# comfy-creator/Comfy-Gen-Server

Measured on AMD Instinct MI355X. Metric: images/sec (whole node) + sec/image, SDXL 1024 20-step Euler-a at 1/2/4/8 MI355X, higher is better.
Workload: dtype bf16; 1 GPU; model=sdxl-base, global_batch=8, seq_len=16384, resolution=1024, sampler_steps=20, sampler=euler_ancestral, unet_batch_per_gpu=16, parallelism=dp1, pipelined=True

## Files before the change

comfy_gen_server_amd/_native.py:

```python
from __future__ import annotations

import ctypes
import glob
import os
import threading

_HERE = os.path.dirname(os.path.abspath(__file__))
LIB_DIR = os.path.join(_HERE, "lib")
_lock = threading.Lock()
_kernels = None
_kernels_err = None


def kernel_lib_path() -> str:
    return os.environ.get("CGS_KERNELS_SO") or os.path.join(LIB_DIR, "libcgs_kernels.so")


def load_kernels():
    global _kernels, _kernels_err
    if _kernels is not None or _kernels_err is not None:
        return _kernels
    with _lock:
        if _kernels is not None or _kernels_err is not None:
            return _kernels
# ... 100 lines not shown
    "cgs_step_param": [_P, _I, _P, _I, _I, _P, _P],
    "cgs_step_advance": [_P, _P],
    "cgs_vae_out_u8": [_P, _P, _L, _P],
    "cgs_conv2d_nhwc_ex": [_P, _P, _I, _P, _P, _P, _P, _I, _I, _I, _I, _I, _I, _I, _I, _I, _I, _I, _I, _P],
    "cgs_region_accumulate": [_P, _P, _P, _I, _P, _I, _I, _I, _I, _I, _I, _I, _I, _I, _L, _L, _L, _L, _I, _L, _L,
                              _L, _L, _I, _F, _P],
    "cgs_region_normalize": [_P, _P, _P, _L, _I, _P],
    "cgs_clip_embed": [_P, _P, _P, _P, _I, _I, _I, _I, _I, _P],
    "cgs_pooled_gather": [_P, _P, _P, _I, _I, _I, _I, _P],
    "cgs_layernorm_stats": [_P, _P, _I, _I, _F, _I, _P],
    "cgs_gemm_bf16_lnfold": [_P, _P, _P, _P, _P, _P, _I, _I, _I, _L, _L, _L, _I, _P, _L, _P],
    "cgs_gemm_bf16_lnfold_v": [_P, _P, _P, _P, _P, _P, _I, _I, _I, _L, _L, _L, _I, _P, _L, _I, _P],
    "cgs_v7_ws_bytes": [_I, _I, _I],
    "cgs_v7_set_dbg": [_I],
    "cgs_v6_set_mode": [_I],
    "cgs_attn_set_prio": [_I],
    "cgs_gn_set_blocks": [_I],
    "cgs_conv_smalln_set_lds": [_I],
    "cgs_attn_set_kv2_rows": [_I],
    "cgs_grn_set_rows": [_I],
    "cgs_flash_attn_fwd_ks": [_P, _P, _P, _P, _I, _I, _I, _I, _L, _L, _L, _L, _L, _L, _L, _L, _F, _I, _P, _P, _P],
    "cgs_flash_attn_fwd_kv2": [_P, _P, _P, _P, _P, _P, _I, _I, _I, _I, _I, _L, _L, _L, _L, _L, _L, _L, _L, _L, _L, _L, _L, _F, _P],
    "cgs_conv2d_nhwc_gns": [_P, _P, _I, _P, _P, _P, _P, _I, _I, _I, _I, _I, _I, _I, _I, _I, _I, _I, _I, _P, _P],
    "cgs_groupnorm_band_stats": [_P, _P, _I, _P, _P, _P, _I, _I, _I, _I, _I, _P],
    "cgs_groupnorm_apply_stats": [_P, _P, _I, _P, _P, _P, _P, _P, _P, _I, _I, _I, _I, _I, _I, _P],
    "cgs_groupnorm_nhwc_part": [_P, _P, _P, _P, _P, _P, _P, _I, _I, _I, _I, _I, _F, _I, _I, _P],
    "cgs_groupnorm_nhwc_part_pld": [_P, _P, _P, _P, _P, _I, _P, _P, _I, _I, _I, _I, _I, _F, _I, _I, _P],
    "cgs_groupnorm_nhwc_ws_pld": [_P, _P, _P, _P, _P, _I, _P, _I, _I, _I, _I, _F, _I, _I, _P],
    "cgs_groupnorm_nhwc_dual_pld": [_P, _P, _I, _P, _P, _P, _P, _I, _P, _I, _I, _I, _I, _F, _I, _I, _P],
    "cgs_gemm_bf16_v7ws": [_P, _P, _P, _P, _P, _I, _I, _I, _L, _L, _L, _L, _I, _F, _P, _L, _P],
    "cgs_conv2d_nhwc_v7ws": [_P, _P, _I, _P, _P, _P, _P, _I, _I, _I, _I, _I, _I, _I, _I, _I, _I, _I, _I, _P, _L, _P],
    "cgs_fourier_filter": [_P, _P, _P, _I, _I, _I, _I, _L, _L, _L, _L, _L, _L, _L, _L, _I, _F, _I, _P],
    "cgs_tome_match": [_P, _P, _P, _P, _P, _I, _I, _I, _I, _L, _L, _L, _L, _I, _P],
    "cgs_grn_nhwc_v2": [_P, _P, _P, _P, _P, _I, _I, _I, _I, _I, _P],
    "cgs_grn_slices": [_I, _I, _I],
    "cgs_bgemm_f32": [_P, _P, _P, _I, _I, _I, _I, _L, _L, _L, _L, _L, _L, _L, _L, _F, _I, _I, _P],
    "cgs_softmax2_f32_bf16": [_P, _P, _L, _I, _L, _L, _P],
    "cgs_transpose_bf16": [_P, _P, _I, _I, _L, _L, _P],
    "cgs_abort_stream_capture": [_P],
    "cgs_channel_affine2": [_P, _P, _P, _L, _P, _I, _I, _I, _F, _I, _P],
    "cgs_gemm_bf16_w6": [_P, _P, _P, _P, _P, _P, _P, _I, _I, _I, _L, _L, _L, _L, _I, _F, _I, _I, _I, _I, _P],
    "cgs_gemm_w6_ok": [_I, _I, _I, _L, _L, _L, _L, _I, _I],
    "cgs_gemm_skinny_ws": [_P, _P, _P, _P, _P, _I, _I, _I, _L, _L, _L, _L, _I, _F, _P, _L, _P],
    "cgs_gemm_skinny_ws_bytes": [_I, _I, _I],
    "cgs_gemm_bf16_rowstats": [_P, _P, _P, _P, _P, _I, _I, _I, _L, _L, _L, _L, _I, _F, _P, _P],
    "cgs_gemm_bf16_rowstats_v": [_P, _P, _P, _P, _P, _I, _I, _I, _L, _L, _L, _L, _I, _F, _P, _I, _P],
# ... 54 lines not shown
```

comfy_gen_server_amd/csrc/kernels/conv.hip:

```cpp
#include "common.h"
#include <stdlib.h>
#include "mfma_core.h"
#include "mfma_pp.h"
#include "mfma_pp160.h"
#include "mfma_ppk.h"

#define EPI_BIAS 1
#define EPI_RESIDUAL 2
#define CONV_UP2X 16
#ifndef CGS_CONV_PFE
#define CGS_CONV_PFE 0
#endif

typedef __attribute__((address_space(3))) void lds_void;

__device__ __attribute__((aligned(16))) unsigned char g_conv_zero_page[256];

struct ConvArgs {
  const u16* in;
  const u16* in2;
  const u16* w;
  const u16* bias;
  const u16* res;
  u16* out;
  int N, H, W, Cin, C1, Cout, kh, kw, stride, pad, Ho, Wo;
  int flags;
  int tiles_n;
// ... 417 lines not shown
        for (int kx = 0; kx < a->kw; ++kx)
          if (ry && (unsigned)(px + kx) < (unsigned)a->W) m |= 1u << (ky * a->kw + kx);
      }
    }
    vm[s] = m;
    const unsigned ch = 16u * (unsigned)pp::src_chunk8(s & 1);
    pb1[s] = pix * (2u * (unsigned)a->C1) + ch;
    pb2[s] = pix * (2u * (unsigned)(a->Cin - a->C1)) + ch;
  }
  __device__ __forceinline__ void dma(int s, int k0, unsigned char* dst) const {
    const unsigned kq = (unsigned)k0 >> 6;
    const unsigned tap = __umulhi(kq, a->cq_magic) + (a->cq_magic ? 0u : kq);
    const int ci0 = k0 - (int)tap * a->Cin;
    const int ky = (int)((tap * (unsigned)a->kw_m16) >> 16);
    const int kx = (int)tap - ky * a->kw;
    const bool second = ci0 >= a->C1;
    const unsigned cs2 = 2u * (unsigned)(second ? a->Cin - a->C1 : a->C1);
    const unsigned so = (unsigned)(ky * a->W + kx) * cs2 + 2u * (unsigned)(second ? ci0 - a->C1 : ci0);
    const unsigned off = ((second ? pb2[s] : pb1[s]) + so) | (~(vm[s] << (31u - tap)) & 0x80000000u);
    __builtin_amdgcn_raw_ptr_buffer_load_lds(second ? r2 : r1, (lds_void*)dst, 16, off, 0, 0, 0);
  }
};

struct ConvGatherKU {
  static constexpr bool kOwnDMA = true;
  const ConvArgs* a;
  uint32_t pb[4], vm[4];
  int py[4], px[4];
  __amdgpu_buffer_rsrc_t r1;
  __device__ __forceinline__ void make(long long n_img, unsigned pixels) {
    r1 = __builtin_amdgcn_make_buffer_rsrc((void*)(a->in + n_img * pixels * a->C1), 0,
                                           (int)(pixels * (unsigned)a->C1 * 2u), 0x00020000);
  }
  __device__ __forceinline__ void init() {
    if (!a->img_rsrc) make(0, (unsigned)(a->N * a->H * a->W));
  }
  __device__ __forceinline__ void tile(int m0) {
    if (a->img_rsrc) make(m0 / (a->Ho * a->Wo), (unsigned)(a->H * a->W));
  }
  __device__ __forceinline__ void setup(int s, int row) {
    const int M = a->N * a->Ho * a->Wo;
    const bool ok = row < M;
    row = ok ? row : M - 1;
    const int hw = a->Ho * a->Wo;
    const int n = row / hw;
    const int rem = row - n * hw;
// ... 139 lines not shown
  conv_magic(a);
  if (g_conv_v6_ld != 1 && kd) conv_run<conv_nhwc_v5k_kernel<true>>(a, nwg, pp::THREADS, pp::LDS, stream);
  else conv_run<conv_nhwc_v5k_kernel<false>>(a, nwg, pp::THREADS, pp::LDS, stream);
}

static int conv_pq_loader(ConvArgs& a) {
  const int kd = conv_kd(a);
  int ld = conv_fast_ok(a) ? (kd ? 2 : 1) : ((a.flags & CONV_UP2X) && kd ? 3 : 0);
  if (g_conv_v6_ld >= 0 && g_conv_v6_ld < ld) ld = ld == 3 ? 0 : g_conv_v6_ld;
  a.img_rsrc = ld >= 2 && kd == 2;
  if (ld) conv_magic(a);
  return ld;
}
template <typename F>
static void with_loader(int ld, F f) {
  if (ld == 3) f(std::integral_constant<int, 3>{});
  else if (ld == 2) f(std::integral_constant<int, 2>{});
  else if (ld == 1) f(std::integral_constant<int, 1>{});
  else f(std::integral_constant<int, 0>{});
}

template <int LD>
using ConvLoaderFor = typename std::conditional<
    LD == 3, ConvGatherKU,
    typename std::conditional<LD == 2, ConvGatherKD,
                              typename std::conditional<LD == 1, ConvGatherK<true>, ConvGatherA8>::type>::type>::type;
template <int LD, int DS = 0, bool GNS = false, int NJ = 5, int PFE = CGS_CONV_PFE>
__global__ __launch_bounds__(512) __attribute__((amdgpu_waves_per_eu(2, 2))) void conv_nhwc_v6_kernel(ConvArgs a) {
  extern __shared__ __attribute__((aligned(16))) unsigned char smem[];
  const int M = a.N * a.Ho * a.Wo;
  const int K = a.kh * a.kw * a.Cin;
  ConvLoaderFor<LD> al;
  al.a = &a;
  if constexpr (LD >= 2) al.init();
  mc::Epi e = conv_epi(a);
  e.gnp = a.gnp;
  e.hw = a.Ho * a.Wo;
  pq::run<decltype(al), false, DS, GNS, false, false, false, PFE, NJ>(al, a.w, K, M, a.Cout, K, e, smem,
                                                                              (M + pq::BM - 1) / pq::BM, a.tiles_n,
                                                                              a.group_m);
}

template <int LD>
__global__ __launch_bounds__(256) __attribute__((amdgpu_waves_per_eu(2, 2))) void conv_nhwc_v6w4_kernel(ConvArgs a) {
  extern __shared__ __attribute__((aligned(16))) unsigned char smem[];
  const int M = a.N * a.Ho * a.Wo;
  const int K = a.kh * a.kw * a.Cin;
  ConvLoaderFor<LD> al;
  al.a = &a;
// ... 25 lines not shown
  if (a.gnp) n128 = false;
  const long long T = conv_tiles(a, pq::BM, n128 ? pq::Geo<4>::BN : pq::BN);
  const int grid = (int)(T < num_cus() ? T : num_cus());
  const int ds = v6_conv_ds();
  with_loader(conv_pq_loader(a), [&](auto lc) {
    constexpr int L = decltype(lc)::value;
    if (a.gnp) {
      conv_v6_launch<L, 51, true>(a, grid, stream);
      return;
    }
    if (n128) {
      conv_v6_launch<L, 51, false, 4, 0>(a, grid, stream);
      return;
    }
    switch (ds) {
      case 0: conv_v6_launch<L, 0>(a, grid, stream); break;
      case 3: conv_v6_launch<L, 3>(a, grid, stream); break;
      case 17: conv_v6_launch<L, 17>(a, grid, stream); break;
      case 19: conv_v6_launch<L, 19>(a, grid, stream); break;
      case 1: conv_v6_launch<L, 1>(a, grid, stream); break;
      default: conv_v6_launch<L, 51>(a, grid, stream);
    }
  });
}

template <int LOADER>
__global__ __launch_bounds__(512) __attribute__((amdgpu_waves_per_eu(2, 2))) void conv_nhwc_v7_kernel(ConvArgs a) {
  extern __shared__ __attribute__((aligned(16))) unsigned char smem[];
  const int M = a.N * a.Ho * a.Wo;
  const int K = a.kh * a.kw * a.Cin;
  typename std::conditional<LOADER == 2, ConvGatherKL,
                            typename std::conditional<LOADER == 1, ConvGatherKB, ConvGatherA8>::type>::type al;
  al.a = &a;
  if constexpr (LOADER >= 1) al.init();
  mc::Epi e = conv_epi(a);
  ppk::run<false>(al, a.w, K, M, a.Cout, K, e, smem, (M + ppk::BM - 1) / ppk::BM, a.tiles_n, a.group_m, a.sp);
}

static void conv_v7_go(ConvArgs& a, hipStream_t stream, void* ws = nullptr, long long ws_bytes = 0) {
  const int K = a.kh * a.kw * a.Cin;
  const long long T = conv_tiles(a, ppk::BM, ppk::BN);
  a.sp = ppk::Split{0, 1, nullptr, nullptr, 0};
  long long U = T;
  if (ws && ws_bytes >= ppk::split_ws_bytes(T, K / ppk::BK, num_cus())) {
    a.sp.S = ppk::split_plan(T, K / ppk::BK, num_cus(), a.sp.t_full);
    if (a.sp.S > 1) {
// ... 217 lines not shown
static bool smalln_lds() {
  if (g_smalln_lds < 0) g_smalln_lds = getenv("CGS_SMALLN_LDS") ? atoi(getenv("CGS_SMALLN_LDS")) != 0 : 1;
  return g_smalln_lds != 0;
}
CGS_EXPORT void cgs_conv_smalln_set_lds(int on) { g_smalln_lds = on != 0; }

static int conv_smalln_launch(const ConvArgs& a, hipStream_t stream) {
  const long long nwg = (long long)a.N * ((a.Ho + 15) / 16) * ((a.Wo + 15) / 16);
  if (nwg > 0x7fffffffLL || nwg < 1) return (int)hipErrorInvalidValue;
  if (smalln_lds() && a.kh == 3 && a.kw == 3 && a.stride == 1 && a.pad == 1 && !(a.flags & CONV_UP2X) &&
      a.in2 == nullptr && a.Cin % 32 == 0 && a.Ho == a.H && a.Wo == a.W && a.Cout <= 16 &&
      (long long)a.H * a.W * a.Cin < (1ll << 31)) {
    conv_nhwc_smalln_lds_kernel<<<(unsigned)nwg, 256, 0, stream>>>(a);
    return (int)hipGetLastError();
  }
  if (a.kh == 3 && a.kw == 3) conv_nhwc_smalln_kernel<3><<<(unsigned)nwg, 256, 0, stream>>>(a);
  else if (a.kh == 1 && a.kw == 1) conv_nhwc_smalln_kernel<1><<<(unsigned)nwg, 256, 0, stream>>>(a);
  else conv_nhwc_smalln_kernel<0><<<(unsigned)nwg, 256, 0, stream>>>(a);
  return (int)hipGetLastError();
}

static int conv_launch(ConvArgs& a, hipStream_t stream, int variant = -2, void* ws = nullptr, long long ws_bytes = 0) {
  if (variant == -2) variant = g_conv_variant;
  if (a.Cout <= 16 && (variant != 2 || a.Cin % 64 || (a.in2 && a.C1 % 64))) return conv_smalln_launch(a, stream);
  if (variant != 2 && a.Cout % 8 == 0) return conv_v3_launch(a, variant, stream, ws, ws_bytes);
  if (a.Cout >= 1024) conv_run<conv_nhwc_v2_kernel<256>>(a, conv_tiles(a, 256, 256), 512, 4 * 64 * (256 + 256), stream);
  else conv_run<conv_nhwc_v2_kernel<128>>(a, conv_tiles(a, 256, 128), 512, 4 * 64 * (256 + 128), stream);
  return (int)hipGetLastError();
}

static ConvArgs conv_args(const void* x, const void* x2, int C1, const void* w, const void* bias, const void* res,
                          void* out, int N, int H, int W, int Cin, int Cout, int kh, int kw, int stride, int pad,
                          int Ho, int Wo, int flags) {
  return ConvArgs{(const u16*)x, (const u16*)x2, (const u16*)w, (const u16*)bias, (const u16*)res, (u16*)out, N, H, W,
                  Cin, x2 ? C1 : Cin, Cout, kh, kw, stride, pad, Ho, Wo,
                  (bias ? EPI_BIAS : 0) | (res ? EPI_RESIDUAL : 0) | (flags & CONV_UP2X), 0, g_conv_group};
}

static bool conv_shape_ok(const ConvArgs& a) {
  return !(a.Cin % 32 || (a.in2 && a.C1 % 32) || a.Cout < 1 ||
           (a.Cout % 8 && a.Cout > 16 && (a.Cin % 64 || (a.in2 && a.C1 % 64))));
}

CGS_EXPORT int cgs_conv2d_nhwc(const void* x, const void* w, const void* bias, const void* res, void* out, int N, int H,
                               int W, int Cin, int Cout, int kh, int kw, int stride, int pad, int Ho, int Wo,
                               hipStream_t stream) {
// ... 19 lines not shown
                                   const void* res, void* out, int N, int H, int W, int Cin, int Cout, int kh, int kw,
                                   int stride, int pad, int Ho, int Wo, int flags, int variant, int act,
                                   float act_param, hipStream_t stream) {
  ConvArgs a = conv_args(x, x2, C1, w, bias, res, out, N, H, W, Cin, Cout, kh, kw, stride, pad, Ho, Wo, flags);
  if (!conv_shape_ok(a) || Cout <= 16 || Cout % 8 || (variant != 3 && variant != 4 && variant != 8) ||
      act < CGS_ACT_NONE || act > CGS_ACT_LEAKY_RELU)
    return (int)hipErrorInvalidValue;
  a.act = act;
  a.act_param = act_param;
  return conv_launch(a, stream, variant);
}

CGS_EXPORT int cgs_conv2d_nhwc_gns(const void* x, const void* x2, int C1, const void* w, const void* bias,
                                   const void* res, void* out, int N, int H, int W, int Cin, int Cout, int kh, int kw,
                                   int stride, int pad, int Ho, int Wo, int flags, float* gnp, hipStream_t stream) {
  ConvArgs a = conv_args(x, x2, C1, w, bias, res, out, N, H, W, Cin, Cout, kh, kw, stride, pad, Ho, Wo, flags);
  if (!gnp || ((uintptr_t)gnp % 16) || (Ho * Wo) % 256 || Cout % 8 || !conv_variant_ok(a, 6))
    return (int)hipErrorInvalidValue;
  a.gnp = gnp;
  conv_v6_go(a, stream);
  return (int)hipGetLastError();
}

CGS_EXPORT int cgs_conv2d_nhwc_v7ws(const void* x, const void* x2, int C1, const void* w, const void* bias,
                                    const void* res, void* out, int N, int H, int W, int Cin, int Cout, int kh, int kw,
                                    int stride, int pad, int Ho, int Wo, int flags, void* ws, long long ws_bytes,
                                    hipStream_t stream) {
  ConvArgs a = conv_args(x, x2, C1, w, bias, res, out, N, H, W, Cin, Cout, kh, kw, stride, pad, Ho, Wo, flags);
  return conv_shape_ok(a) ? conv_launch(a, stream, 7, ws, ws_bytes) : (int)hipErrorInvalidValue;
}
```

comfy_gen_server_amd/csrc/kernels/mfma_pp160.h:

```cpp
#pragma once
#include "common.h"
#include "mfma_core.h"
#include "mfma_pp.h"

namespace pq {

typedef uint32_t u32x4v __attribute__((ext_vector_type(4)));
typedef uint32_t u32x2v __attribute__((ext_vector_type(2)));
__device__ __forceinline__ void untracked_load(u32x4v& d, const void* p) {
  asm volatile("global_load_dwordx4 %0, %1, off" : "=v"(d) : "v"(p));
}
__device__ __forceinline__ void untracked_load(u32x2v& d, const void* p) {
  asm volatile("global_load_dwordx2 %0, %1, off" : "=v"(d) : "v"(p));
}

constexpr int BM = 256, BN = 160, BK = 64;
constexpr int THREADS = 512;
constexpr int A_BYTES = BM * 128;
constexpr int B_BYTES = BN * 128;
constexpr int STAGE = A_BYTES + B_BYTES;
constexpr int LDS = 3 * STAGE;
template <int NJ, int NI = 4, int W = 8>
struct Geo {
  static constexpr int GW = 16 * NJ, BN = GW * (W / 4);
  static constexpr int BM = 64 * NI;
  static constexpr int PR = 8 * W;
  static constexpr int NA = BM / PR;
  static constexpr int A_BYTES = BM * 128;
  static constexpr int B_BYTES = BN * 128, STAGE = A_BYTES + B_BYTES, LDS = 3 * STAGE;
  static constexpr int NBG = (BN + PR - 1) / PR;
  static constexpr int REM = BN % PR;
  static constexpr bool B_HALF = REM != 0;
};

template <int NJ = 5>
__device__ __forceinline__ int b_col160(int r) {
  constexpr int GW = 16 * NJ;
  const int g = r >= GW, l = r - GW * g, j = l >> 4, q = l & 15;
  if (j >= 4) return GW * g + 64 + q;
  return GW * g + 32 * (j >> 1) + 8 * (q >> 2) + 4 * (j & 1) + (q & 3);
// ... 85 lines not shown
#pragma unroll
        for (int g = 0; g < 4; ++g) dma_a(g, kt, slot);
      } else {
#pragma unroll
        for (int g = 0; g < 3; ++g) dma_b(g, kt, slot);
      }
    } else {
      if (part == 0) {
        dma_a(0, kt, slot);
        dma_a(1, kt, slot);
        dma_b(0, kt, slot);
      } else {
        dma_a(2, kt, slot);
        dma_a(3, kt, slot);
        dma_b(1, kt, slot);
        dma_b(2, kt, slot);
      }
    }
  };
  auto stage = [&](int kt, int slot) {
    stage_part(0, kt, slot);
    if constexpr ((DS & 3) != 0) stage_part(1, kt, slot);
  };
  auto wait_tile = [&]() {
    if (!Gm::B_HALF || wave < Gm::REM / 8) mc::wait_vmcnt<Gm::NA + Gm::NBG>();
    else mc::wait_vmcnt<Gm::NA + Gm::NBG - 1>();
  };

  f32x4 acc[NI][NJ];
  const int fr = lane & 15, fq = lane >> 4;
  bf16x8 af[NI], bfr[NJ];
  auto read_frags = [&](const unsigned char* S, int kk) {
#pragma unroll
    for (int i = 0; i < NI; ++i) {
      const int r = wm * (16 * NI) + 16 * i + fr;
      const int c = (4 * kk + fq) ^ ((r >> 1) & 7);
      af[i] = *reinterpret_cast<const bf16x8*>(S + r * 128 + 16 * c);
    }
    const unsigned char* SB = S + A_BYTESv;
#pragma unroll
    for (int j = 0; j < NJ; ++j) {
      const int r = grp * GW + 16 * j + fr;
      const int c = (4 * kk + fq) ^ ((r >> 1) & 7);
      bfr[j] = *reinterpret_cast<const bf16x8*>(SB + r * 128 + 16 * c);
    }
  };
  auto mma = [&]() {
// ... 292 lines not shown
  using T0 = std::false_type;
  using T1 = std::true_type;
  auto epilogue = [&](int m0, int n0) {
    if constexpr (LN) {
      if (hb) epilogue_t(m0, n0, T1{}, T0{});
      else epilogue_t(m0, n0, T0{}, T0{});
      return;
    }
    if (hr) {
      if (hb) epilogue_t(m0, n0, T1{}, T1{});
      else epilogue_t(m0, n0, T0{}, T1{});
    } else {
      if (hb) epilogue_t(m0, n0, T1{}, T0{});
      else epilogue_t(m0, n0, T0{}, T0{});
    }
  };

  int l = base_l;
  int m0, n0;
  coords(l, m0, n0);
  setup(m0, n0);
  stage(0, 0);
  stage(nk > 1 ? 1 : 0, 1);
  wait_tile();
  pp::barrier();
  if (NW == 8 && grp == 1) pp::barrier();

  int slot = 0;
  while (true) {
    const int ln = l + G;
    const bool has_next = ln < T;
    int nm0 = 0, nn0 = 0;
    if (has_next) coords(ln, nm0, nn0);
#pragma unroll
    for (int i = 0; i < NI; ++i)
#pragma unroll
      for (int j = 0; j < NJ; ++j) acc[i][j] = f32x4{0.f, 0.f, 0.f, 0.f};
    auto ktile = [&](int kt, bool PF) {
      const unsigned char* S = smem + slot * STAGE;
      const int slot2 = slot >= 1 ? slot - 1 : 2;
      const int kst = kt + 2 < nk ? kt + 2 : (has_next ? kt + 2 - nk : nk - 1);
      if (kt + 2 == nk && has_next) setup(nm0, nn0);
      if constexpr ((DS & 4) != 0) stage_part(0, kst, slot2);
      read_frags(S, 0);
      if constexpr ((DS & 4) == 0) stage_part(0, kst, slot2);
      if constexpr ((DS & 16) == 0) pp::wait_lgkm0();
      pp::barrier();
      mma();
      pp::barrier();
      if constexpr ((DS & 4) != 0) stage_part(1, kst, slot2);
      read_frags(S, 1);
      if constexpr ((DS & 4) == 0) stage_part(1, kst, slot2);
      wait_tile();
      if (PFE && PF) prefetch(m0, n0, hb, PFE == 1 && hr);
      pp::wait_lgkm0();
      pp::barrier();
      mma();
      pp::barrier();
      slot = slot == 2 ? 0 : slot + 1;
    };
    if constexpr (PFE == 2) {
      for (int kt = 0; kt < nk; ++kt) ktile(kt, kt == nk - 2);
    } else if constexpr (PFE) {
      for (int kt = 0; kt < nk - 2; ++kt) ktile(kt, false);
      ktile(nk - 2, true);
      ktile(nk - 1, false);
    } else {
      for (int kt = 0; kt < nk; ++kt) ktile(kt, false);
    }
    epilogue(m0, n0);
    if (!has_next) break;
    l = ln;
    m0 = nm0;
    n0 = nn0;
  }
  if (NW == 8 && grp == 0) pp::barrier();
// ... 5 lines not shown
```

comfy_gen_server_amd/ops/core.py:

```python
from __future__ import annotations

import collections
import math
import os

import numpy as np
import torch
import torch.nn.functional as F

from .. import _native
from . import autotune
from . import f32 as _f32
from .dispatch import backend_for, count, vendor_fallback

_DT = {torch.float32: 0, torch.bfloat16: 1, torch.float16: 2}

EPI_BIAS = 1
EPI_RESIDUAL = 2
EPI_GEGLU = 4
EPI_SILU_IN = 8
EPI_LNFOLD = 8
EPI_GELU = 32
EPI_F32OUT = 16

# ... 790 lines not shown
    pd = padding[0] if isinstance(padding, (tuple, list)) else padding
    y = sc.conv2d(lambda xx, _: _conv2d(xx, weight, bias, st, pd, None, weight_nhwc, groups, upsample2x, None),
                  x, weight.shape[2], st, pd, upsample2x, x2)
    if residual is not None:
        y = y + residual
    return y.contiguous(memory_format=torch.channels_last) if y.is_cuda else y


def upconv_tap_weights(weight: torch.Tensor) -> torch.Tensor:
    Cout, Cin = weight.shape[:2]
    G = (Cout + 15) // 16
    w = weight.new_zeros((G * 16, Cin, 9))
    w[:Cout] = weight.reshape(Cout, Cin, 9)
    return w.view(G, 16, Cin, 9).permute(0, 3, 1, 2).contiguous().view(G * 144, Cin)


def _upconv_use_taps(N, H, W, Cin, Cout, cached) -> bool:
    mode = os.environ.get("CGS_UPCONV_TAPS", "")
    if mode in ("0", "1"):
        return mode == "1"
    return cached and Cin >= 256 and Cout >= 32 and N * H * W * Cin * Cout * 36 >= (1 << 27)


CONV_VARIANTS = {"v2": 2, "v3": 3, "v4": 4, "v5": 5, "v6": 6, "v7": 7, "v8": 8, "v6n128": 18, "v6w4": 21, "auto": -2}
_FUSED_ACT_CONV = ("v3", "v4", "v8")


def _conv_operands(xc, x2c, w_nhwc, bias, res, out, kh, kw, stride, pad, flags):
    N, C1, H, W = xc.shape
    _, Cout, Ho, Wo = out.shape
    return (xc.data_ptr(), _ptr(x2c), C1, w_nhwc.data_ptr(), _ptr(bias), _ptr(res), out.data_ptr(), N, H, W,
            C1 + (0 if x2c is None else x2c.shape[1]), Cout, kh, kw, stride, pad, Ho, Wo, flags)


def _conv2d_act(x, weight, bias, stride, padding, residual, weight_nhwc, groups, upsample2x, x2, act, act_param):
    if act not in ACT_CODES:
        raise ValueError(f"unknown activation {act!r} (one of {sorted(ACT_CODES)})")
    st = stride[0] if isinstance(stride, (tuple, list)) else stride
    pd = padding[0] if isinstance(padding, (tuple, list)) else padding

    def split():
        y = conv2d(x, weight, bias, st, pd, weight_nhwc=weight_nhwc, groups=groups, upsample2x=upsample2x, x2=x2)
        y = activation(y, act, act_param, inplace=True)
        return y if residual is None else y + residual.to(y.dtype)

    Cout, _, kh, kw = weight.shape
    C1 = x.shape[1]
# ... 62 lines not shown
        x2c = None if x2 is None else x2.contiguous(memory_format=torch.channels_last)
        Hl, Wl = (2 * H, 2 * W) if upsample2x else (H, W)
        Ho = (Hl + 2 * padding - kh) // stride + 1
        Wo = (Wl + 2 * padding - kw) // stride + 1
        xc = x.contiguous(memory_format=torch.channels_last)
        r = None
        if residual is not None:
            r = residual.contiguous(memory_format=torch.channels_last)
        flags = 16 if upsample2x else 0

        def run(variant):
            out = torch.empty((N, Cout, Ho, Wo), device=x.device, dtype=x.dtype,
                              memory_format=torch.channels_last)
            pre = _conv_operands(xc, x2c, weight_nhwc, bias, r, out, kh, kw, stride, padding, flags)
            ws = _v7_ws(N * Ho * Wo, Cout, kh * kw * Cin, x.device) if variant == 7 else None
            if ws is not None:
                _check(_lib().cgs_conv2d_nhwc_v7ws(*pre, ws.data_ptr(), ws.numel(), _stream()), "cgs_conv2d_nhwc_v7ws")
            else:
                _check(_lib().cgs_conv2d_nhwc_v(*pre, variant, _stream()), "cgs_conv2d_nhwc")
            return out

        variant = -2
        M = N * Ho * Wo
        if M * Cout * Cin * kh * kw >= (1 << 27) and Cout > 16:
            cands = [("v4", lambda: run(4))]
            if Cout % 8 == 0:
                cands.append(("v8", lambda: run(8)))
            if Cin % 64 == 0:
                cands += [("v7", lambda: run(7)), ("v5", lambda: run(5)), ("v6", lambda: run(6)),
                          ("v2", lambda: run(2))]
                if Cout % 128 == 0 and Cout % 160 and kh * kw * Cin >= 128:
                    cands.append(("v6n128", lambda: run(18)))
                if Cout % 80 == 0 and kh * kw * Cin >= 128 and M <= 32768:
                    cands.append(("v6w4", lambda: run(21)))
            choice = autotune.choose(("conv", N, H, W, Cin, Cout, kh, stride, padding, flags, int(r is not None))
                                     + ((("dual", C1),) if x2c is not None else ()), cands, default="auto")
            variant = CONV_VARIANTS[choice]
        if (upsample2x and single and r is None and not gn_stats and kh == 3 and kw == 3 and stride == 1
                and padding == 1 and Cout % 8 == 0 and weight.dtype == x.dtype
                and _native.has_kernel("cgs_upconv_taps_nhwc")):
            def run_taps():
                wt = weight_taps() if callable(weight_taps) else weight_taps
                if wt is None:
                    wt = upconv_tap_weights(weight)
                out = torch.empty((N, Cout, Ho, Wo), device=x.device, dtype=x.dtype,
                                  memory_format=torch.channels_last)
                _check(_lib().cgs_upconv_taps_nhwc(xc.data_ptr(), wt.data_ptr(), _ptr(bias), out.data_ptr(), N, H, W,
                                                   Cin, Cout, _stream()), "cgs_upconv_taps_nhwc")
                return out

            if _upconv_use_taps(N, H, W, Cin, Cout, weight_taps is not None):
                return run_taps()
        if (gn_stats and variant == 6 and _GNS and (Ho * Wo) % 256 == 0 and Cin % 64 == 0 and C1 % 64 == 0
                and Cout % 8 == 0 and kh * kw * Cin >= 128 and (bias is None or bias.data_ptr() % 8 == 0)
                and _native.has_kernel("cgs_conv2d_nhwc_gns")):
            out = torch.empty((N, Cout, Ho, Wo), device=x.device, dtype=x.dtype, memory_format=torch.channels_last)
            part = torch.empty(N * (Ho * Wo // 64) * Cout * 2, device=x.device, dtype=torch.float32)
            _check(_lib().cgs_conv2d_nhwc_gns(*_conv_operands(xc, x2c, weight_nhwc, bias, r, out, kh, kw, stride,
                                                              padding, flags), part.data_ptr(), _stream()),
                   "cgs_conv2d_nhwc_gns")
            out._cgs_gnpart = (part, out.data_ptr())
            return out
        return run(variant)
    if upsample2x:
        x = upsample_nearest2x(x)
    if be == "torch":
        count("conv", "torch")
        y = F.conv2d(x.float(), weight.float(), None if bias is None else bias.float(), stride, padding,
                     groups=groups)
        if residual is not None:
            y = y + residual.float()
        return y.to(x.dtype)
    vendor_fallback("conv", f"dtype {x.dtype}, groups={groups}, Cin={x.shape[1]}, Cout={Cout}")
    y = F.conv2d(x, weight, bias, stride, padding, groups=groups)
    if residual is not None:
        y = y + residual
    return y


_CT_TAPS = ((3, 1), (2, 0))


def conv_transpose_phase_weights(weight: torch.Tensor):
# ... 1308 lines not shown
```

Before: 3.465 images/s.

## Add halo-patch 3x3 conv kernel reusing LDS input tile across all nine taps

Adds a new v6p conv kernel for 3x3 stride-1 convolutions. It loads an 18x18 halo input patch per channel slab into LDS once and reuses it for all nine taps, instead of re-gathering the im2col A operand for every tap. Weight tiles for each tap are streamed through a triple-buffered slot ring, and the kernel supports the fused GroupNorm partial-stats epilogue. It is enabled by default for a fixed set of SDXL UNet shapes whenever variant 6 is chosen, and it is also added as an autotune candidate. A probe loader variant that skips A loads after the first tap is also added, but it is not on the default path.

```diff
diff --git a/comfy_gen_server_amd/_native.py b/comfy_gen_server_amd/_native.py
--- a/comfy_gen_server_amd/_native.py
+++ b/comfy_gen_server_amd/_native.py
@@ -146,6 +146,8 @@
     "cgs_flash_attn_fwd_ks": [_P, _P, _P, _P, _I, _I, _I, _I, _L, _L, _L, _L, _L, _L, _L, _L, _F, _I, _P, _P, _P],
     "cgs_flash_attn_fwd_kv2": [_P, _P, _P, _P, _P, _P, _I, _I, _I, _I, _I, _L, _L, _L, _L, _L, _L, _L, _L, _L, _L, _L, _L, _F, _P],
     "cgs_conv2d_nhwc_gns": [_P, _P, _I, _P, _P, _P, _P, _I, _I, _I, _I, _I, _I, _I, _I, _I, _I, _I, _I, _P, _P],
+    "cgs_conv2d_nhwc_gns_v": [_P, _P, _I, _P, _P, _P, _P, _I, _I, _I, _I, _I, _I, _I, _I, _I, _I, _I, _I, _P, _I, _P],
+    "cgs_conv2d_nhwc_probe": [_P, _P, _P, _P, _P, _I, _I, _I, _I, _I, _I, _I, _I, _I, _I, _I, _P],
     "cgs_groupnorm_band_stats": [_P, _P, _I, _P, _P, _P, _I, _I, _I, _I, _I, _P],
     "cgs_groupnorm_apply_stats": [_P, _P, _I, _P, _P, _P, _P, _P, _P, _I, _I, _I, _I, _I, _I, _P],
     "cgs_groupnorm_nhwc_part": [_P, _P, _P, _P, _P, _P, _P, _I, _I, _I, _I, _I, _F, _I, _I, _P],
diff --git a/comfy_gen_server_amd/csrc/kernels/conv.hip b/comfy_gen_server_amd/csrc/kernels/conv.hip
--- a/comfy_gen_server_amd/csrc/kernels/conv.hip
+++ b/comfy_gen_server_amd/csrc/kernels/conv.hip
@@ -3,6 +3,7 @@
 #include "mfma_core.h"
 #include "mfma_pp.h"
 #include "mfma_pp160.h"
+#include "mfma_pp160p.h"
 #include "mfma_ppk.h"
 
 #define EPI_BIAS 1
@@ -466,6 +467,14 @@
   }
 };
 
+struct ConvGatherKD1 : ConvGatherKD {
+  static constexpr bool kTapProbe = true;
+  __device__ __forceinline__ bool has_a(int k0) const { return k0 < a->Cin; }
+  __device__ __forceinline__ void dma(int s, int k0, unsigned char* dst) const {
+    if (has_a(k0)) ConvGatherKD::dma(s, k0, dst);
+  }
+};
+
 struct ConvGatherKU {
   static constexpr bool kOwnDMA = true;
   const ConvArgs* a;
@@ -651,9 +660,10 @@
 
 template <int LD>
 using ConvLoaderFor = typename std::conditional<
+    LD == 4, ConvGatherKD1, typename std::conditional<
     LD == 3, ConvGatherKU,
     typename std::conditional<LD == 2, ConvGatherKD,
-                              typename std::conditional<LD == 1, ConvGatherK<true>, ConvGatherA8>::type>::type>::type;
+                              typename std::conditional<LD == 1, ConvGatherK<true>, ConvGatherA8>::type>::type>::type>::type;
 template <int LD, int DS = 0, bool GNS = false, int NJ = 5, int PFE = CGS_CONV_PFE>
 __global__ __launch_bounds__(512) __attribute__((amdgpu_waves_per_eu(2, 2))) void conv_nhwc_v6_kernel(ConvArgs a) {
   extern __shared__ __attribute__((aligned(16))) unsigned char smem[];
@@ -725,6 +735,31 @@
       default: conv_v6_launch<L, 51>(a, grid, stream);
     }
   });
+}
+
+template <bool GNS>
+__global__ __launch_bounds__(512) __attribute__((amdgpu_waves_per_eu(2, 2))) void conv_nhwc_v6p_kernel(ConvArgs a) {
+  extern __shared__ __attribute__((aligned(16))) unsigned char smem[];
+  mc::Epi e = conv_epi(a);
+  e.gnp = a.gnp;
+  e.hw = a.H * a.W;
+  pq::run_patch<GNS>(a.in, a.N, a.H, a.W, a.Cin, a.w, a.Cout, e, smem, a.tiles_n);
+}
+
+static bool conv_patch_ok(const ConvArgs& a) {
+  const long long units = (long long)a.N * ((a.H + 15) / 16) * ((a.W + 15) / 16) * ((a.Cout + pq::BN - 1) / pq::BN);
+  return a.kh == 3 && a.kw == 3 && a.stride == 1 && a.pad == 1 && !a.in2 && !(a.flags & CONV_UP2X) && !a.act &&
+         a.Cin % 64 == 0 && a.Cout % 8 == 0 && a.Ho == a.H && a.Wo == a.W && (uintptr_t)a.bias % 8 == 0 &&
+         (long long)a.H * a.W * a.Cin * 2 < (1ll << 31) && units < (1ll << 31) &&
+         (!a.gnp || (a.H % 16 == 0 && a.W % 16 == 0));
+}
+
+static void conv_v6p_go(ConvArgs& a, hipStream_t stream) {
+  a.tiles_n = (a.Cout + pq::BN - 1) / pq::BN;
+  const long long T = (long long)a.N * ((a.H + 15) / 16) * ((a.W + 15) / 16) * a.tiles_n;
+  const long long grid = T < num_cus() ? T : num_cus();
+  if (a.gnp) conv_run<conv_nhwc_v6p_kernel<true>>(a, grid, pq::THREADS, pq::P_LDS, stream);
+  else conv_run<conv_nhwc_v6p_kernel<false>>(a, grid, pq::THREADS, pq::P_LDS, stream);
 }
 
 template <int LOADER>
@@ -988,6 +1023,11 @@
 
 static int conv_launch(ConvArgs& a, hipStream_t stream, int variant = -2, void* ws = nullptr, long long ws_bytes = 0) {
   if (variant == -2) variant = g_conv_variant;
+  if (variant == 22) {
+    if (!conv_patch_ok(a)) return (int)hipErrorInvalidValue;
+    conv_v6p_go(a, stream);
+    return (int)hipGetLastError();
+  }
   if (a.Cout <= 16 && (variant != 2 || a.Cin % 64 || (a.in2 && a.C1 % 64))) return conv_smalln_launch(a, stream);
   if (variant != 2 && a.Cout % 8 == 0) return conv_v3_launch(a, variant, stream, ws, ws_bytes);
   if (a.Cout >= 1024) conv_run<conv_nhwc_v2_kernel<256>>(a, conv_tiles(a, 256, 256), 512, 4 * 64 * (256 + 256), stream);
@@ -1053,6 +1093,33 @@
   return (int)hipGetLastError();
 }
 
+CGS_EXPORT int cgs_conv2d_nhwc_gns_v(const void* x, const void* x2, int C1, const void* w, const void* bias,
+                                     const void* res, void* out, int N, int H, int W, int Cin, int Cout, int kh, int kw,
+                                     int stride, int pad, int Ho, int Wo, int flags, float* gnp, int variant,
+                                     hipStream_t stream) {
+  if (variant != 22)
+    return variant == 6 ? cgs_conv2d_nhwc_gns(x, x2, C1, w, bias, res, out, N, H, W, Cin, Cout, kh, kw, stride, pad,
+                                              Ho, Wo, flags, gnp, stream)
+                        : (int)hipErrorInvalidValue;
+  ConvArgs a = conv_args(x, x2, C1, w, bias, res, out, N, H, W, Cin, Cout, kh, kw, stride, pad, Ho, Wo, flags);
+  if (!gnp || ((uintptr_t)gnp % 16) || !conv_shape_ok(a)) return (int)hipErrorInvalidValue;
+  a.gnp = gnp;
+  if (!conv_patch_ok(a)) return (int)hipErrorInvalidValue;
+  conv_v6p_go(a, stream);
+  return (int)hipGetLastError();
+}
+
+CGS_EXPORT int cgs_conv2d_nhwc_probe(const void* x, const void* w, const void* bias, const void* res, void* out, int N,
+                                     int H, int W, int Cin, int Cout, int kh, int kw, int stride, int pad, int Ho,
+                                     int Wo, hipStream_t stream) {
+  ConvArgs a = conv_args(x, nullptr, Cin, w, bias, res, out, N, H, W, Cin, Cout, kh, kw, stride, pad, Ho, Wo, 0);
+  if (!conv_shape_ok(a) || Cout % 8 || Cout <= 16 || !conv_variant_ok(a, 6) || conv_pq_loader(a) != 2)
+    return (int)hipErrorInvalidValue;
+  const long long T = conv_tiles(a, pq::BM, pq::BN);
+  conv_v6_launch<4, 51>(a, (int)(T < num_cus() ? T : num_cus()), stream);
+  return (int)hipGetLastError();
+}
+
 CGS_EXPORT int cgs_conv2d_nhwc_v7ws(const void* x, const void* x2, int C1, const void* w, const void* bias,
                                     const void* res, void* out, int N, int H, int W, int Cin, int Cout, int kh, int kw,
                                     int stride, int pad, int Ho, int Wo, int flags, void* ws, long long ws_bytes,
diff --git a/comfy_gen_server_amd/csrc/kernels/mfma_pp160.h b/comfy_gen_server_amd/csrc/kernels/mfma_pp160.h
--- a/comfy_gen_server_amd/csrc/kernels/mfma_pp160.h
+++ b/comfy_gen_server_amd/csrc/kernels/mfma_pp160.h
@@ -16,6 +16,10 @@
 
 constexpr int BM = 256, BN = 160, BK = 64;
 constexpr int THREADS = 512;
+template <class T, class = void>
+struct tap_probe : std::false_type {};
+template <class T>
+struct tap_probe<T, std::void_t<decltype(T::kTapProbe)>> : std::true_type {};
 constexpr int A_BYTES = BM * 128;
 constexpr int B_BYTES = BN * 128;
 constexpr int STAGE = A_BYTES + B_BYTES;
@@ -147,7 +151,14 @@
     stage_part(0, kt, slot);
     if constexpr ((DS & 3) != 0) stage_part(1, kt, slot);
   };
-  auto wait_tile = [&]() {
+  auto wait_tile = [&](int kin) {
+    if constexpr (tap_probe<AL>::value) {
+      if (!al.has_a(kin * BK)) {
+        if (!Gm::B_HALF || wave < Gm::REM / 8) mc::wait_vmcnt<Gm::NBG>();
+        else mc::wait_vmcnt<Gm::NBG - 1>();
+        return;
+      }
+    }
     if (!Gm::B_HALF || wave < Gm::REM / 8) mc::wait_vmcnt<Gm::NA + Gm::NBG>();
     else mc::wait_vmcnt<Gm::NA + Gm::NBG - 1>();
   };
@@ -486,7 +497,7 @@
   setup(m0, n0);
   stage(0, 0);
   stage(nk > 1 ? 1 : 0, 1);
-  wait_tile();
+  wait_tile(nk > 1 ? 1 : 0);
   pp::barrier();
   if (NW == 8 && grp == 1) pp::barrier();
 
@@ -515,7 +526,7 @@
       if constexpr ((DS & 4) != 0) stage_part(1, kst, slot2);
       read_frags(S, 1);
       if constexpr ((DS & 4) == 0) stage_part(1, kst, slot2);
-      wait_tile();
+      wait_tile(kst);
       if (PFE && PF) prefetch(m0, n0, hb, PFE == 1 && hr);
       pp::wait_lgkm0();
       pp::barrier();
diff --git a/comfy_gen_server_amd/csrc/kernels/mfma_pp160p.h b/comfy_gen_server_amd/csrc/kernels/mfma_pp160p.h
--- /dev/null
+++ b/comfy_gen_server_amd/csrc/kernels/mfma_pp160p.h
@@ -0,0 +1,302 @@
+#pragma once
+#include "mfma_pp160.h"
+
+namespace pq {
+
+constexpr int PATCH = 16, PATCH_W = PATCH + 2, PATCH_PIX = PATCH_W * PATCH_W;
+constexpr int PA_ROUNDS = 6;
+constexpr int PA_BYTES = PA_ROUNDS * 8 * 1024;
+constexpr int PB_BYTES = Geo<5>::B_BYTES;
+constexpr int P_LDS = 2 * PA_BYTES + 3 * PB_BYTES;
+
+struct PatchUnit {
+  int n, y0, x0, n0, pi;
+};
+
+template <bool GNS>
+__device__ __forceinline__ void run_patch(const u16* __restrict__ X, int NB, int H, int Wd, int Cin,
+                                          const u16* __restrict__ Wt, int N, const mc::Epi& e, unsigned char* smem,
+                                          int tiles_n) {
+  using Gm = Geo<5>;
+  constexpr int NI = 4, NJ = 5, GW = Gm::GW, BN = Gm::BN;
+  const int tid = threadIdx.x;
+  const int lane = tid & 63;
+  const int wave = __builtin_amdgcn_readfirstlane(tid >> 6);
+  const int grp = wave >> 2;
+  const int wm = wave & 3;
+  const int nslab = Cin / 64;
+  const long long ldw = 9ll * Cin;
+  const int tiles_x = (Wd + PATCH - 1) / PATCH, tiles_y = (H + PATCH - 1) / PATCH;
+  const int ppi = tiles_x * tiles_y;
+  const int T = NB * ppi * tiles_n;
+  const int G = gridDim.x;
+  const int base_l = xcd_remap(blockIdx.x, G);
+  if (base_l >= T) return;
+
+  auto decode = [&](int l) {
+    PatchUnit u;
+    const int pg = l / tiles_n;
+    u.n0 = (l - pg * tiles_n) * BN;
+    u.n = pg / ppi;
+    u.pi = pg - u.n * ppi;
+    const int ty = u.pi / tiles_x;
+    u.y0 = ty * PATCH;
+    u.x0 = (u.pi - ty * tiles_x) * PATCH;
+    return u;
+  };
+
+  unsigned char* const SA = smem;
+  unsigned char* const SB = smem + 2 * PA_BYTES;
+
+  uint32_t voff[PA_ROUNDS];
+  __amdgpu_buffer_rsrc_t ra;
+  auto a_setup = [&](const PatchUnit& u) {
+    ra = __builtin_amdgcn_make_buffer_rsrc((void*)(X + (long long)u.n * H * Wd * Cin), 0, H * Wd * Cin * 2, 0x00020000);
+#pragma unroll
+    for (int r = 0; r < PA_ROUNDS; ++r) {
+      const int d = (r * 8 + wave) * 64 + lane;
+      const int p = d >> 3, c = d & 7;
+      const int py = p / PATCH_W, px = p - py * PATCH_W;
+      const int iy = u.y0 - 1 + py, ix = u.x0 - 1 + px;
+      const bool ok = p < PATCH_PIX && (unsigned)iy < (unsigned)H && (unsigned)ix < (unsigned)Wd;
+      voff[r] = ok ? (uint32_t)(((iy * Wd + ix) * Cin + 8 * (c ^ (p & 7))) * 2) : 0x80000000u;
+    }
+  };
+  auto dma_a = [&](int r, int slab, int buf) {
+    __builtin_amdgcn_raw_ptr_buffer_load_lds(ra, (mc_lds_void*)(SA + buf * PA_BYTES + (r * 8 + wave) * 1024), 16,
+                                             voff[r], slab * 128, 0, 0);
+  };
+
+  const int lrow = tid >> 3, lch = tid & 7;
+  const u16* bsrc[3];
+  auto b_setup = [&](int n0) {
+#pragma unroll
+    for (int g = 0; g < 3; ++g) {
+      const int r = g * 64 + lrow;
+      int n = n0 + b_col160<5>(r < BN ? r : BN - 1);
+      n = n < N ? n : N - 1;
+      bsrc[g] = Wt + (long long)n * ldw + 8 * (lch ^ ((r >> 1) & 7));
+    }
+  };
+  auto dma_b = [&](int g, int tap, int slab, int slot) {
+    if (g == 2 && wave >= 4) return;
+    mc::lds_dma16((const void*)(bsrc[g] + tap * Cin + slab * 64), SB + slot * PB_BYTES + wave * 1024 + g * 8192);
+  };
+  auto wait_step = [&](auto ac) {
+    constexpr int A = decltype(ac)::value;
+    if (wave < 4) mc::wait_vmcnt<3 + A>();
+    else mc::wait_vmcnt<2 + A>();
+  };
+
+  f32x4 acc[NI][NJ];
+  const int fr = lane & 15, fq = lane >> 4;
+  bf16x8 af[NI], bfr[NJ];
+  const int pbase = 4 * wm * PATCH_W + fr;
+  int abase[8][2], bbase[2];
+#pragma unroll
+  for (int m = 0; m < 8; ++m)
+#pragma unroll
+    for (int kk = 0; kk < 2; ++kk) abase[m][kk] = (pbase + m) * 128 + 16 * ((4 * kk + fq) ^ ((pbase + m) & 7));
+#pragma unroll
+  for (int kk = 0; kk < 2; ++kk)
+    bbase[kk] = 2 * PA_BYTES + (grp * GW + fr) * 128 + 16 * ((4 * kk + fq) ^ (fr >> 1));
+  auto read_frags = [&](int aoff, auto tapc, auto slotc, auto kkc) {
+    constexpr int tapoff = decltype(tapc)::value, slot = decltype(slotc)::value, kk = decltype(kkc)::value;
+    mc::static_for<0, NI>([&](auto ic) {
+      constexpr int i = decltype(ic)::value, c = i * PATCH_W + tapoff;
+      af[i] = *reinterpret_cast<const bf16x8*>(smem + (aoff + abase[c & 7][kk]) + (c >> 3) * 1024);
+    });
+    mc::static_for<0, NJ>([&](auto jc) {
+      constexpr int j = decltype(jc)::value;
+      bfr[j] = *reinterpret_cast<const bf16x8*>(smem + bbase[kk] + (slot * PB_BYTES + j * 2048));
+    });
+  };
+  auto mma = [&]() {
+    __builtin_amdgcn_s_setprio(1);
+#pragma unroll
+    for (int i = 0; i < NI; ++i)
+#pragma unroll
+      for (int j = 0; j < NJ; ++j) acc[i][j] = __builtin_amdgcn_mfma_f32_16x16x32_bf16(bfr[j], af[i], acc[i][j], 0, 0, 0);
+    __builtin_amdgcn_s_setprio(0);
+  };
+
+  auto colj = [&](int j) { return j < 4 ? 32 * (j >> 1) + 8 * fq + 4 * (j & 1) : 64 + 4 * fq; };
+  auto epilogue_t = [&](const PatchUnit& u, auto has_bias_c, auto has_res_c) {
+    constexpr bool HB = decltype(has_bias_c)::value, HR = decltype(has_res_c)::value;
+    const int n_w = u.n0 + grp * GW;
+    const int x = u.x0 + fr, yw = u.y0 + 4 * wm;
+    const long long img_row = (long long)u.n * H * Wd;
+    auto row_of = [&](int ib, long long& row) {
+      const int y = yw + ib;
+      row = img_row + (long long)y * Wd + x;
+      return y < H && x < Wd;
+    };
+    float4 bv[NJ];
+#pragma unroll
+    for (int j = 0; j < NJ; ++j) {
+      int col = n_w + colj(j);
+      col = col < N ? col : N - 4;
+      bv[j] = HB ? unpack4_bf16(*reinterpret_cast<const uint2*>(e.bias + col)) : float4{0.f, 0.f, 0.f, 0.f};
+    }
+    uint2 rw[NI][NJ];
+    if (HR) {
+#pragma unroll
+      for (int i = 0; i < NI; ++i) {
+        long long row;
+        if (!row_of(i, row)) row = img_row;
+        const u16* rrow = e.R + row * e.ldr;
+#pragma unroll
+        for (int p = 0; p < 2; ++p) {
+          int col = n_w + 32 * p + 8 * fq;
+          col = col < N ? col : N - 8;
+          const uint4 w4 = *reinterpret_cast<const uint4*>(rrow + col);
+          rw[i][2 * p] = uint2{w4.x, w4.y};
+          rw[i][2 * p + 1] = uint2{w4.z, w4.w};
+        }
+        int col = n_w + 64 + 4 * fq;
+        col = col < N ? col : N - 4;
+        rw[i][4] = *reinterpret_cast<const uint2*>(rrow + col);
+      }
+    }
+    uint2 pk[NI][NJ];
+#pragma unroll
+    for (int i = 0; i < NI; ++i)
+#pragma unroll
+      for (int j = 0; j < NJ; ++j) {
+        float v0 = acc[i][j][0] * e.alpha + bv[j].x, v1 = acc[i][j][1] * e.alpha + bv[j].y;
+        float v2 = acc[i][j][2] * e.alpha + bv[j].z, v3 = acc[i][j][3] * e.alpha + bv[j].w;
+        if (HR) {
+          const float4 rv = unpack4_bf16(rw[i][j]);
+          v0 += rv.x; v1 += rv.y; v2 += rv.z; v3 += rv.w;
+        }
+        pk[i][j] = pack4_bf16(v0, v1, v2, v3);
+      }
+#pragma unroll
+    for (int i = 0; i < NI; ++i) {
+      long long row;
+      const bool ok = row_of(i, row);
+#pragma unroll
+      for (int p = 0; p < 2; ++p) {
+        const int col = n_w + 32 * p + 8 * fq;
+        if (ok && col < N)
+          *reinterpret_cast<uint4*>(e.C + row * e.ldc + col) =
+              uint4{pk[i][2 * p].x, pk[i][2 * p].y, pk[i][2 * p + 1].x, pk[i][2 * p + 1].y};
+      }
+    }
+#pragma unroll
+    for (int i = 0; i < NI; i += 2) {
+      const auto rx = __builtin_amdgcn_permlane16_swap(pk[i][4].x, pk[i + 1][4].x, false, false);
+      const auto ry = __builtin_amdgcn_permlane16_swap(pk[i][4].y, pk[i + 1][4].y, false, false);
+      long long row;
+      const bool ok = row_of(i + (fq & 1), row);
+      const int col = n_w + 64 + 8 * (fq >> 1);
+      if (ok && col < N) *reinterpret_cast<uint4*>(e.C + row * e.ldc + col) = uint4{rx[0], ry[0], rx[1], ry[1]};
+    }
+    if constexpr (GNS) {
+      const int nbk = (H * Wd) >> 6;
+      float* dst = e.gnp + (size_t)(u.n * nbk + u.pi * 4 + wm) * N * 2;
+#pragma unroll
+      for (int j = 0; j < NJ; ++j) {
+        float4 v[NI];
+#pragma unroll
+        for (int i = 0; i < NI; ++i) v[i] = unpack4_bf16(pk[i][j]);
+        float4 mu = v[0];
+#pragma unroll
+        for (int i = 1; i < NI; ++i) { mu.x += v[i].x; mu.y += v[i].y; mu.z += v[i].z; mu.w += v[i].w; }
+        constexpr float inv = 1.f / 64.f;
+        mu = float4{row16_sum(mu.x) * inv, row16_sum(mu.y) * inv, row16_sum(mu.z) * inv, row16_sum(mu.w) * inv};
+        float4 q = float4{0.f, 0.f, 0.f, 0.f};
+#pragma unroll
+        for (int i = 0; i < NI; ++i) {
+          const float dx = v[i].x - mu.x, dy = v[i].y - mu.y, dz = v[i].z - mu.z, dw = v[i].w - mu.w;
+          q.x += dx * dx; q.y += dy * dy; q.z += dz * dz; q.w += dw * dw;
+        }
+        q = float4{row16_sum(q.x), row16_sum(q.y), row16_sum(q.z), row16_sum(q.w)};
+        const int col = n_w + colj(j);
+        if (fr == 0 && col < N) {
+          float4* d4 = reinterpret_cast<float4*>(dst + (size_t)col * 2);
+          d4[0] = float4{mu.x, q.x, mu.y, q.y};
+          d4[1] = float4{mu.z, q.z, mu.w, q.w};
+        }
+      }
+    }
+  };
+  using T0 = std::false_type;
+  using T1 = std::true_type;
+  const bool hb = (e.flags & MC_EPI_BIAS) != 0, hr = (e.flags & MC_EPI_RESIDUAL) != 0;
+  auto epilogue = [&](const PatchUnit& u) {
+    if (hr) {
+      if (hb) epilogue_t(u, T1{}, T1{});
+      else epilogue_t(u, T0{}, T1{});
+    } else {
+      if (hb) epilogue_t(u, T1{}, T0{});
+      else epilogue_t(u, T0{}, T0{});
+    }
+  };
+
+  int l = base_l;
+  PatchUnit u = decode(l);
+  a_setup(u);
+  b_setup(u.n0);
+#pragma unroll
+  for (int r = 0; r < PA_ROUNDS; ++r) dma_a(r, 0, 0);
+#pragma unroll
+  for (int g = 0; g < 3; ++g) dma_b(g, 0, 0, 0);
+#pragma unroll
+  for (int g = 0; g < 3; ++g) dma_b(g, 1, 0, 1);
+  wait_step(std::integral_constant<int, 0>{});
+  pp::barrier();
+  if (grp == 1) pp::barrier();
+
+  int abuf = 0;
+  while (true) {
+    const int ln = l + G;
+    const bool has_next = ln < T;
+    const PatchUnit nu = has_next ? decode(ln) : u;
+#pragma unroll
+    for (int i = 0; i < NI; ++i)
+#pragma unroll
+      for (int j = 0; j < NJ; ++j) acc[i][j] = f32x4{0.f, 0.f, 0.f, 0.f};
+    for (int s = 0; s < nslab; ++s) {
+      const bool last = s == nslab - 1;
+      if (last && has_next) a_setup(nu);
+      const int sn = last ? 0 : s + 1;
+      const int aoff = abuf * PA_BYTES;
+      mc::static_for<0, 9>([&](auto tc) {
+        constexpr int t = decltype(tc)::value;
+        constexpr int tapoff = (t / 3) * PATCH_W + t % 3;
+        constexpr int t2 = (t + 2) % 9, slot2 = (t + 2) % 3;
+        constexpr bool AR = t >= 1 && t <= PA_ROUNDS;
+        const int s2 = t + 2 < 9 ? s : sn;
+        if constexpr (t == 7) {
+          if (last && has_next) b_setup(nu.n0);
+        }
+        using Tap = std::integral_constant<int, tapoff>;
+        using Slot = std::integral_constant<int, t % 3>;
+        read_frags(aoff, Tap{}, Slot{}, std::integral_constant<int, 0>{});
+        dma_b(0, t2, s2, slot2);
+        if constexpr (AR) dma_a(t - 1, sn, abuf ^ 1);
+        pp::barrier();
+        mma();
+        pp::barrier();
+        read_frags(aoff, Tap{}, Slot{}, std::integral_constant<int, 1>{});
+        dma_b(1, t2, s2, slot2);
+        dma_b(2, t2, s2, slot2);
+        wait_step(std::integral_constant<int, AR ? 1 : 0>{});
+        pp::wait_lgkm0();
+        pp::barrier();
+        mma();
+        pp::barrier();
+      });
+      abuf ^= 1;
+    }
+    epilogue(u);
+    if (!has_next) break;
+    l = ln;
+    u = nu;
+  }
+  if (grp == 0) pp::barrier();
+  mc::wait_vmcnt<0>();
+}
+
+}
diff --git a/comfy_gen_server_amd/ops/core.py b/comfy_gen_server_amd/ops/core.py
--- a/comfy_gen_server_amd/ops/core.py
+++ b/comfy_gen_server_amd/ops/core.py
@@ -836,7 +836,27 @@
     return cached and Cin >= 256 and Cout >= 32 and N * H * W * Cin * Cout * 36 >= (1 << 27)
 
 
-CONV_VARIANTS = {"v2": 2, "v3": 3, "v4": 4, "v5": 5, "v6": 6, "v7": 7, "v8": 8, "v6n128": 18, "v6w4": 21, "auto": -2}
+def _conv_patch_ok(x, x2, bias, Cin, Cout, kh, kw, stride, padding, upsample2x) -> bool:
+    H, W = x.shape[2], x.shape[3]
+    return (kh == 3 and kw == 3 and stride == 1 and padding == 1 and x2 is None and not upsample2x
+            and x.dtype == torch.bfloat16 and Cin % 64 == 0 and Cout % 8 == 0 and H * W * Cin * 2 < (1 << 31)
+            and (bias is None or bias.data_ptr() % 8 == 0) and _native.has_kernel("cgs_conv2d_nhwc_gns_v"))
+
+
+def _conv_use_patch(variant: int, N, H, W, Cin, Cout) -> bool:
+    mode = os.environ.get("CGS_CONV_PATCH", "")
+    if mode in ("0", "1"):
+        return mode == "1"
+    return variant == 6 and (N, H, W, Cin, Cout) in _PATCH_SHAPES
+
+
+_PATCH_SHAPES = frozenset(
+    [(16, 128, 128, c, 320) for c in (320, 640, 960)] + [(16, 64, 64, c, 640) for c in (320, 640, 960, 1280, 1920)]
+    + [(16, 32, 32, c, 1280) for c in (640, 1280, 1920, 2560)])
+
+
+CONV_VARIANTS = {"v2": 2, "v3": 3, "v4": 4, "v5": 5, "v6": 6, "v7": 7, "v8": 8, "v6n128": 18, "v6w4": 21, "v6p": 22,
+                 "auto": -2}
 _FUSED_ACT_CONV = ("v3", "v4", "v8")
 
 
@@ -945,6 +965,7 @@
 
         variant = -2
         M = N * Ho * Wo
+        patch_ok = _conv_patch_ok(xc, x2c, bias, Cin, Cout, kh, kw, stride, padding, upsample2x)
         if M * Cout * Cin * kh * kw >= (1 << 27) and Cout > 16:
             cands = [("v4", lambda: run(4))]
             if Cout % 8 == 0:
@@ -956,9 +977,15 @@
                     cands.append(("v6n128", lambda: run(18)))
                 if Cout % 80 == 0 and kh * kw * Cin >= 128 and M <= 32768:
                     cands.append(("v6w4", lambda: run(21)))
+                if patch_ok:
+                    cands.append(("v6p", lambda: run(22)))
             choice = autotune.choose(("conv", N, H, W, Cin, Cout, kh, stride, padding, flags, int(r is not None))
                                      + ((("dual", C1),) if x2c is not None else ()), cands, default="auto")
             variant = CONV_VARIANTS[choice]
+        if patch_ok and variant != 22 and _conv_use_patch(variant, N, H, W, Cin, Cout):
+            variant = 22
+        elif variant == 22 and os.environ.get("CGS_CONV_PATCH", "") == "0":
+            variant = 6
         if (upsample2x and single and r is None and not gn_stats and kh == 3 and kw == 3 and stride == 1
                 and padding == 1 and Cout % 8 == 0 and weight.dtype == x.dtype
                 and _native.has_kernel("cgs_upconv_taps_nhwc")):
@@ -974,14 +1001,16 @@
 
             if _upconv_use_taps(N, H, W, Cin, Cout, weight_taps is not None):
                 return run_taps()
-        if (gn_stats and variant == 6 and _GNS and (Ho * Wo) % 256 == 0 and Cin % 64 == 0 and C1 % 64 == 0
+        if (gn_stats and variant in (6, 22) and _GNS and (Ho * Wo) % 256 == 0 and Cin % 64 == 0 and C1 % 64 == 0
                 and Cout % 8 == 0 and kh * kw * Cin >= 128 and (bias is None or bias.data_ptr() % 8 == 0)
                 and _native.has_kernel("cgs_conv2d_nhwc_gns")):
             out = torch.empty((N, Cout, Ho, Wo), device=x.device, dtype=x.dtype, memory_format=torch.channels_last)
             part = torch.empty(N * (Ho * Wo // 64) * Cout * 2, device=x.device, dtype=torch.float32)
-            _check(_lib().cgs_conv2d_nhwc_gns(*_conv_operands(xc, x2c, weight_nhwc, bias, r, out, kh, kw, stride,
-                                                              padding, flags), part.data_ptr(), _stream()),
-                   "cgs_conv2d_nhwc_gns")
+            pre = _conv_operands(xc, x2c, weight_nhwc, bias, r, out, kh, kw, stride, padding, flags)
+            if variant == 22 and H % 16 == 0 and W % 16 == 0:
+                _check(_lib().cgs_conv2d_nhwc_gns_v(*pre, part.data_ptr(), 22, _stream()), "cgs_conv2d_nhwc_gns_v")
+            else:
+                _check(_lib().cgs_conv2d_nhwc_gns(*pre, part.data_ptr(), _stream()), "cgs_conv2d_nhwc_gns")
             out._cgs_gnpart = (part, out.data_ptr())
             return out
         return run(variant)
```

Result: faster. 3.578 images/s, median of 6 (+3.3%).
